# rapidsai/cudf

Measured on AMD Instinct MI355X. Metric: rows/sec + achieved HBM GB/s: 1e9-row int64 sort & hash-join, 1/2/4/8 GPU, higher is better.
Workload: dtype int64; 1 GPU; 1e+09-row int64 radix sort (cudf::sort, keys only); rows_per_gpu=1000000000, algo=0, parallelism=1 GPU

## Files before the change

### cudf_amd/csrc/gx_sort.hip

```cpp
#include "gx_common.hpp"
#include <cstdlib>
#include <type_traits>
#include <vector>
#include "gx_scan.hpp"

namespace gx {
namespace sort {

constexpr int BINS       = 256;
constexpr int MAX_PASSES = 8;
constexpr int BT         = 512;
constexpr int NW         = BT / GX_WAVE;
constexpr int NRANGE     = 8;

constexpr int CS_MAXBITS = 15;
constexpr int NB2MAX     = 1024;
constexpr int NB9        = 512;

struct HybridPlan {
  int32_t attempt;
  int32_t ok;
  int32_t shift0;
  int32_t shift2, bits2;
  int32_t nlocal;
  int32_t lshift[MAX_PASSES], lbits[MAX_PASSES];
  int32_t need_hist;
  int32_t cell_max;
  int32_t overflow;
  int32_t bad;
  uint32_t plan2_done;
  unsigned long long or_mask, nor_mask;
  uint32_t list_tile0[2][NRANGE + 1];
  uint32_t seg_tile0[2][BINS + 1];
  uint32_t seg_start[2][BINS], seg_count[2][BINS];
  uint32_t max_cell;
  uint32_t hist0[BINS], gbin0[BINS];
  uint32_t rh0[NRANGE][BINS];
  uint32_t rhist[NRANGE][MAX_PASSES][BINS];
  unsigned long long fold_or;
  int32_t fold;
  unsigned long long fold_x;
  alignas(128) uint32_t todo_count;
  uint32_t todo_pad[31];
  int32_t big;
  int32_t lsd_mode;
  uint32_t nbig;
  uint32_t big_pad;
  unsigned long long lsd_n;
  uint32_t bigbucket[BINS];
  uint32_t bigcnt[BINS], bigkeys[BINS];
  uint32_t biglist0[BINS], bigx0[BINS];
  uint32_t cbase[BINS], ccap[BINS];
};
__device__ __forceinline__ uint32_t cell_cap(const HybridPlan& hy, uint32_t b) { return hy.ccap[b] ? hy.ccap[b] : (uint32_t)hy.cell_max; }
__device__ __forceinline__ uint32_t cell_slot(const HybridPlan& hy, uint32_t b, uint32_t d2)
{
  return hy.ccap[b] ? hy.cbase[b] + d2 * hy.ccap[b] : ((b << hy.bits2) + d2) * (uint32_t)hy.cell_max;
}
static inline size_t cell_slack(int cell_max) { return (size_t)(6.0 * __builtin_sqrt((double)cell_max)) + 64 + 16 + 2; }

struct FastPlan {
  int32_t state;
  int32_t cs_bits;
  uint32_t cs_fail;
  uint32_t cs_groups;
  unsigned long long cs_base;
  int32_t fail;
  int32_t stride;
  int32_t hist_ready;
  int32_t slots_ready;
  uint32_t samp[NRANGE][BINS];
  uint32_t slot0[NRANGE][BINS];
  uint32_t cap0[NRANGE][BINS];
  uint32_t reg_tile0[BINS * NRANGE + 1];
  uint32_t reg_start[BINS * NRANGE], reg_count[BINS * NRANGE];
  alignas(128) uint32_t cur0[NRANGE][BINS];
  uint32_t forced_masks;
  unsigned long long forced_or, forced_nor;
  uint32_t ext, nreg;
  uint32_t slot_total;
  uint32_t* x_tile0;
  const uint32_t* x_start;
  const uint32_t* x_count;
  const uint32_t* x_bucket;
};

struct alignas(128) Counter {
  uint32_t v;
  uint32_t pad[31];
};
struct SortCounters {
  Counter tickets[MAX_PASSES];
  Counter ctr[2][NRANGE];
};

constexpr int SP_NSAMP = 16384;
// ... 25 lines not shown
};
struct SpCell {
  unsigned long long lo, w;
  uint32_t mlow;
  int nsh;
};
__device__ __forceinline__ SpCell sp_cell_of(const SplitPlan& sp, uint32_t b) { return SpCell{sp.lo[b], sp.w[b], sp.mlow[b], sp.nsh[b]}; }
__device__ __forceinline__ bool sp_narrow(const SplitPlan& sp, uint32_t b, int bits2) { return sp.nw[b] != 0u && sp.nw[b] <= (1u << bits2) && !sp.eq[b]; }
__device__ __forceinline__ uint32_t sp_cell(uint32_t frac, uint32_t nc) { return __umulhi(frac, nc); }
template <int CL2>
__device__ __forceinline__ uint32_t sp_fine(uint32_t frac, uint32_t nc) { return __umulhi(frac, nc << CL2) & ((1u << CL2) - 1u); }
__device__ __forceinline__ uint32_t sp_warp(uint32_t frac, const uint2* wt)
{
  const uint2 e = wt[frac >> SP_PSH];
  return e.x + __umulhi(frac << (32 - SP_PSH), e.y);
}
__device__ __forceinline__ uint32_t sp_frac(const SpCell& c, unsigned long long key)
{
  const unsigned long long rel = key > c.lo ? key - c.lo : 0ull;
  if (rel >= c.w) return 0xFFFFFFFFu;
  const uint32_t x2 = c.nsh == 63 ? 0u : ((uint32_t)((rel << (33 - c.nsh)) >> 32) & ~1u);
  return x2 + __umulhi(x2, c.mlow);
}
__device__ __forceinline__ uint32_t sp_lut_cell(unsigned long long rel, uint32_t lut_log, uint32_t lshift)
{
  if (lut_log) {
    if (rel == 0) return 0;
    const int e      = 63 - __builtin_clzll(rel);
    const uint32_t m = e >= 6 ? (uint32_t)(rel >> (e - 6)) & 63u : (uint32_t)(rel << (6 - e)) & 63u;
    return (uint32_t)e * 64u + m;
  }
  const unsigned long long c = rel >> lshift;
  return c < (unsigned long long)(SP_NLUT - 1) ? (uint32_t)c : (uint32_t)(SP_NLUT - 1);
}
struct SpLutF {
  unsigned long long nmin, pmin;
  uint32_t nsh, psh;
};
__device__ __forceinline__ SpLutF sp_lutf_of(const SplitPlan& sp) { return SpLutF{sp.f_nmin, sp.f_pmin, sp.f_nsh, sp.f_psh}; }
template <int KIND, int F2 = -1>
__device__ __forceinline__ uint32_t sp_lut_cell_k(unsigned long long key, unsigned long long kmin, uint32_t form, uint32_t lshift, const SpLutF& f)
{
  if (F2 == 1 || (F2 < 0 && form == 2u)) {
    const bool pos             = key >= f.pmin;
    const unsigned long long o = pos ? f.pmin : f.nmin;
    const unsigned long long c = (key > o ? key - o : 0ull) >> (pos ? f.psh : f.nsh);
    return (pos ? (uint32_t)(SP_NLUT / 2) : 0u) + (c < (unsigned long long)(SP_NLUT / 2 - 1) ? (uint32_t)c : (uint32_t)(SP_NLUT / 2 - 1));
  }
  return sp_lut_cell(key >= kmin ? key - kmin : 0ull, form, lshift);
}
template <int KIND, int F2 = -1>
__device__ __forceinline__ uint32_t sp_bucket(const unsigned long long* __restrict__ tab, const uint16_t* __restrict__ lut, unsigned long long key,
                                              uint32_t nsp, unsigned long long kmin, uint32_t lut_log, uint32_t lshift, const SpLutF& lf)
{
  const uint32_t wd            = lut[sp_lut_cell_k<KIND, F2>(key, kmin, lut_log, lshift, lf)];
  uint32_t b                   = wd & 0x1FFu;
  if (wd & 0x8000u) return b;
  const uint32_t inside = (wd >> 9) & 63u;
  if (inside <= 4u) {
    while (b < nsp && tab[b] <= key) ++b;
    return b;
  }
  uint32_t lo = b, hi = inside == 63u ? nsp : b + inside;
  while (lo < hi) {
    const uint32_t mid = (lo + hi) >> 1;
    if (tab[mid] <= key) lo = mid + 1; else hi = mid;
  }
  return lo;
}

struct SortPlan {
  uint32_t hist[MAX_PASSES][BINS];
  uint32_t gbin[MAX_PASSES][BINS];
  int32_t pass_skip[MAX_PASSES];
  int32_t pass_src[MAX_PASSES];
  int32_t pass_dst[MAX_PASSES];
  int32_t num_active;
  int32_t status;
  HybridPlan hy;
  SortCounters cnt;
  FastPlan hf;
  SplitPlan sp;
};

struct Digit0 {
  int shift, fsh;
  uint32_t dm, fhi;
  template <typename KeyT>
  __device__ __forceinline__ uint32_t operator()(KeyT k) const { return ((uint32_t)(k >> shift) & dm) | ((uint32_t)(k >> fsh) & fhi); }
};
__device__ __forceinline__ Digit0 digit0_of(const HybridPlan& hy, int key_bits)
{
  return hy.fold ? Digit0{hy.shift0, key_bits - 8, 0x7Fu, 0x80u} : Digit0{hy.shift0, 0, 0xFFu, 0u};
}
__device__ __forceinline__ int fold_height(unsigned long long fold_or, unsigned long long V, int key_bits)
{
  if (!((V >> (key_bits - 1)) & 1ull)) return 0;
  const int h = fold_or ? 64 - __builtin_clzll(fold_or) : 0;
  return (h >= 7 && h <= key_bits - 10) ? h : 0;
}

template <typename KeyT, int KIND>
__global__ void __launch_bounds__(BT) k_hist_all(const KeyT* __restrict__ in, int64_t n, KeyT desc_mask,
                                                 SortPlan* plan, int64_t range_rows, const KeyT* __restrict__ inB = nullptr)
{
  if (plan->hy.ok && !plan->hy.lsd_mode) return;
  if (plan->hy.lsd_mode) {
    in         = inB;
    n          = (int64_t)plan->hy.lsd_n;
    range_rows = div_up(div_up(n, (int64_t)NRANGE), (int64_t)GX_WAVE) * GX_WAVE;
  }
  const int range      = blockIdx.x % NRANGE;
  const int64_t rbegin = (int64_t)range * range_rows < n ? (int64_t)range * range_rows : n;
  const int64_t rend   = (range == NRANGE - 1) ? n : (rbegin + range_rows < n ? rbegin + range_rows : n);
  constexpr int NPASS = sizeof(KeyT);
  __shared__ uint32_t s_hist[NPASS * BINS];
  __shared__ unsigned long long s_fold[NW];
  for (int i = threadIdx.x; i < NPASS * BINS; i += BT) s_hist[i] = 0;
  __syncthreads();
  const unsigned lane  = lane_id();
  KeyT fold            = 0;
  constexpr int UNROLL = 4;
  const int64_t stride = (int64_t)(gridDim.x / NRANGE) * BT * UNROLL;
  for (int64_t i0 = rbegin + (int64_t)(blockIdx.x / NRANGE) * BT * UNROLL + threadIdx.x; i0 < rend; i0 += stride) {
    KeyT raw[UNROLL];
#pragma unroll
    for (int u = 0; u < UNROLL; ++u) {
      const int64_t i = i0 + (int64_t)u * BT;
      raw[u]          = (i < rend) ? in[i] : KeyT(0);
    }
#pragma unroll
    for (int u = 0; u < UNROLL; ++u) {
      const int64_t i = i0 + (int64_t)u * BT;
      if (i < rend) {
        const KeyT k          = to_sortable<KeyT, KIND>(raw[u], desc_mask);
        if (KIND == K_SIGNED) fold |= (KeyT)(raw[u] ^ (KeyT)(KeyT(0) - (KeyT)(raw[u] >> (8 * sizeof(KeyT) - 1))));
        const uint64_t active = ballot(true);
        const int leader      = __builtin_ctzll(active);
#pragma unroll
        for (int p = 0; p < NPASS; ++p) {
          const uint32_t d  = (uint32_t)(k >> (8 * p)) & 0xFFu;
          const uint32_t d0 = __builtin_amdgcn_readfirstlane(d);
          const uint64_t same = ballot(d == d0);
          if (same == active) {
            if ((int)lane == leader) atomicAdd(&s_hist[p * BINS + d0], (uint32_t)__builtin_popcountll(active));
          } else if (__builtin_popcountll(same) >= 8) {
            if ((int)lane == leader) atomicAdd(&s_hist[p * BINS + d0], (uint32_t)__builtin_popcountll(same));
            else if (d != d0) atomicAdd(&s_hist[p * BINS + d], 1u);
          } else {
            atomicAdd(&s_hist[p * BINS + d], 1u);
          }
        }
      }
    }
  }
  if (KIND == K_SIGNED) {
    const unsigned long long wf = wave_reduce((unsigned long long)fold, [](unsigned long long x, unsigned long long y) { return x | y; });
    if (lane == 0) s_fold[threadIdx.x / GX_WAVE] = wf;
  }
  __syncthreads();
  if (KIND == K_SIGNED && threadIdx.x == 0) {
    unsigned long long f = 0;
    for (int k = 0; k < NW; ++k) f |= s_fold[k];
    if (f & ~__hip_atomic_load(&plan->hy.fold_or, __ATOMIC_RELAXED, __HIP_MEMORY_SCOPE_AGENT)) atomicOr(&plan->hy.fold_or, f);
  }
  for (int i = threadIdx.x; i < NPASS * BINS; i += BT) {
// ... 2435 lines not shown
      }
    }
    __syncthreads();
    uint32_t q  = s_misc[0];
    uint32_t jt = s_misc[1];
    if constexpr (LVL == 2) {
      q  = (uint32_t)__builtin_amdgcn_readfirstlane((int)q);
      jt = (uint32_t)__builtin_amdgcn_readfirstlane((int)jt);
    }
    seg               = q / NRANGE;
    if (LVL == 2 && !hy.bigbucket[seg]) return;
    base              = (int64_t)hf.reg_start[q] + (int64_t)jt * TILE;
    const int64_t rem = (int64_t)hf.reg_count[q] - (int64_t)jt * TILE;
    nvalid            = (int)(rem < (int64_t)TILE ? rem : (int64_t)TILE);
  } else {
    const uint32_t nreg    = hf.nreg;
    const uint32_t* rtile0 = hf.x_tile0;
    if (v >= (int64_t)rtile0[nreg]) return;
    for (uint32_t q = tid; q < nreg; q += BT) {
      const uint32_t lo = rtile0[q], hi = rtile0[q + 1];
      if ((int64_t)lo <= v && v < (int64_t)hi) {
        s_misc[0] = q;
        s_misc[1] = (uint32_t)(v - lo);
      }
    }
    __syncthreads();
    uint32_t q  = s_misc[0];
    uint32_t jt = s_misc[1];
    if constexpr (LVL == 2) {
      q  = (uint32_t)__builtin_amdgcn_readfirstlane((int)q);
      jt = (uint32_t)__builtin_amdgcn_readfirstlane((int)jt);
    }
    seg               = hf.x_bucket[q];
    if (LVL == 2 && !hy.bigbucket[seg]) return;
    base              = (int64_t)hf.x_start[q] + (int64_t)jt * TILE;
    const int64_t rem = (int64_t)hf.x_count[q] - (int64_t)jt * TILE;
    nvalid            = (int)(rem < (int64_t)TILE ? rem : (int64_t)TILE);
  }
  const uint32_t dmask = LVL == 0 ? 0xFFu : ((1u << hy.bits2) - 1u);
  const Digit0 dig     = LVL == 0 ? digit0_of(hy, (int)(8 * sizeof(KeyT))) : Digit0{hy.shift2, 0, dmask, 0u};
  const uint32_t cap_s  = LVL >= 1 ? cell_cap(hy, seg) : 0u;
  const uint32_t base_s = LVL >= 1 ? cell_slot(hy, seg, 0u) : 0u;
  SpCell spc{0ull, 1ull, 0u, 63};
  if (split) {
    if (plan->sp.eq[seg]) {
      if (LVL == 2) return;
      if (tid == 0) s_misc[2] = atomicAdd(&cellcur[seg * NB2MAX], (uint32_t)nvalid);
      __syncthreads();
      const int64_t dst0 = (int64_t)hy.gbin0[seg] + (int64_t)s_misc[2];
#pragma unroll
      for (int j = 0; j < KPT; ++j) {
        const int idx = j * BT + (int)tid;
        if (idx < nvalid) fin[dst0 + idx] = in[base + idx];
      }
      return;
    }
    spc = sp_cell_of(plan->sp, seg);
    if (tid < (unsigned)SP_NPIECE) s_wt[tid] = plan->sp.wt[seg][tid];
  }
  const uint32_t spnc = split ? plan->sp.nc[seg] : 1u;
  auto spdig          = [&](KeyT k) -> uint32_t {
    if constexpr (sizeof(KeyT) == 8) return sp_cell(sp_warp(sp_frac(spc, (unsigned long long)k), s_wt), spnc);
    else return dig(k);
  };
  if (split && sp_narrow(plan->sp, seg, hy.bits2)) {
    if (LVL == 2) return;
    for (int b = tid; b < NB; b += BT) s_cnt[b] = 0;
    __syncthreads();
#pragma unroll
    for (int j = 0; j < KPT; ++j) {
      const int idx   = j * BT + (int)tid;
      const bool live = idx < nvalid;
      const KeyT k    = to_sortable<KeyT, KIND>(in[base + (live ? idx : 0)], desc_mask);
      (void)lds_rank(s_cnt, spdig(k), live);
    }
    __syncthreads();
    for (int b = tid; b < NB; b += BT) {
      const uint32_t c = s_cnt[b];
      if (c) atomicAdd(&cellcur[seg * NB2MAX + b], c);
    }
    return;
  }

  KeyT key[KPT];
  if (nvalid == TILE) {
#pragma unroll
    for (int j = 0; j < KPT; ++j) key[j] = in[base + j * BT + (int)tid];
  } else {
#pragma unroll
    for (int j = 0; j < KPT; ++j) {
      const int idx = j * BT + (int)tid;
      key[j]        = in[base + (idx < nvalid ? idx : 0)];
    }
  }
  for (int b = tid; b < NB; b += BT) s_cnt[b] = 0;
  if constexpr (LVL == 0 && KIND == K_FTOTAL) {
    bool unclean = false;
#pragma unroll
    for (int j = 0; j < KPT; ++j) unclean |= float_unclean<KeyT>(key[j]);
    if (unclean) hf.fail = 1;
  }
  if (LVL == 0) {
    auto mform = [&](KeyT k) -> KeyT {
      if constexpr (KIND == K_FTOTAL) return to_sortable<KeyT, KIND>(k, KeyT(0));
      else return k;
    };
    KeyT vor = mform(key[0]), vnor = (KeyT)~mform(key[0]);
#pragma unroll
    for (int j = 1; j < KPT; ++j) {
      vor |= mform(key[j]);
      vnor |= (KeyT)~mform(key[j]);
    }
    const unsigned long long wo = wave_reduce((unsigned long long)vor, [](unsigned long long x, unsigned long long y) { return x | y; });
    const unsigned long long wn = wave_reduce((unsigned long long)vnor, [](unsigned long long x, unsigned long long y) { return x | y; });
    if (lane_id() == 0) {
      s_red[tid / GX_WAVE]      = wo;
      s_red[NW + tid / GX_WAVE] = wn;
    }
    if (KIND == K_SIGNED && hy.fold) {
      KeyT vf = 0;
#pragma unroll
      for (int j = 0; j < KPT; ++j) vf |= (KeyT)(key[j] ^ (KeyT)(KeyT(0) - (KeyT)(key[j] >> (8 * sizeof(KeyT) - 1))));
      const unsigned long long wf = wave_reduce((unsigned long long)vf, [](unsigned long long x, unsigned long long y) { return x | y; });
      if (lane_id() == 0 && (wf & ~__hip_atomic_load(&hy.fold_x, __ATOMIC_RELAXED, __HIP_MEMORY_SCOPE_AGENT))) atomicOr(&hy.fold_x, wf);
    }
  }
  __syncthreads();
  if (LVL == 0 && tid == 0) {
    unsigned long long o = 0, no = 0;
    for (int k = 0; k < NW; ++k) {
      o |= s_red[k];
      no |= s_red[NW + k];
    }
    if (o & ~__hip_atomic_load(&hy.or_mask, __ATOMIC_RELAXED, __HIP_MEMORY_SCOPE_AGENT)) atomicOr(&hy.or_mask, o);
    if (no & ~__hip_atomic_load(&hy.nor_mask, __ATOMIC_RELAXED, __HIP_MEMORY_SCOPE_AGENT)) atomicOr(&hy.nor_mask, no);
  }
  constexpr bool RANK16 = sizeof(KeyT) == 4;
  uint32_t packed[RANK16 ? KPT / 2 : KPT];
  if constexpr (RANK16) {
#pragma unroll
    for (int j = 0; j < KPT / 2; ++j) packed[j] = 0;
  }
  auto rank_all = [&](auto&& digf) {
#pragma unroll
    for (int j = 0; j < KPT; ++j) {
      const bool live  = j * BT + (int)tid < nvalid;
      const KeyT k     = to_sortable<KeyT, KIND>(key[j], desc_mask);
      const uint32_t d = digf(k);
      const uint32_t r = lds_rank(s_cnt, d, live);
      if constexpr (RANK16) packed[j >> 1] |= r << (16 * (j & 1));
      else packed[j] = (d << 16) | r;
    }
  };
  if (split) rank_all(spdig); else rank_all(dig);
  __syncthreads();
  uint32_t c[BPT], g[BPT], sbase[BPT], scap[BPT];
  bool skip[BPT];
  uint32_t csum = 0;
#pragma unroll
  for (int k = 0; k < BPT; ++k) {
    const uint32_t bin = tid * BPT + k;
    c[k] = g[k] = sbase[k] = scap[k] = 0;
    skip[k] = false;
    if (bin < (uint32_t)NB) {
      c[k] = s_cnt[bin];
      if (LVL == 0) {
        sbase[k] = hf.slot0[seg][bin];
        scap[k]  = hf.cap0[seg][bin];
        if (c[k]) g[k] = atomicAdd(&hf.cur0[seg][bin], c[k]);
      } else if (LVL == 1 && bin <= dmask) {
        sbase[k] = base_s + bin * cap_s;
        scap[k]  = cap_s;
        if (c[k]) g[k] = atomicAdd(&cellcur[seg * NB2MAX + bin], c[k]);
      } else if (LVL == 2 && bin <= dmask) {
        const uint32_t total = cellcur[seg * NB2MAX + bin];
        if (total > cap_s) {
          sbase[k] = xoff[seg * NB2MAX + bin];
          scap[k]  = total;
          if (c[k]) g[k] = atomicAdd(&rescur[seg * NB2MAX + bin], c[k]);
        } else {
          skip[k] = true;
        }
      }
      csum += c[k];
    }
  }
  uint32_t st = block_exclusive_scan<BT>(csum, 0u, SumOp(), s_scan, (uint32_t*)nullptr);
  bool spilled = false;
#pragma unroll
  for (int k = 0; k < BPT; ++k) {
    const uint32_t bin = tid * BPT + k;
    if (bin < (uint32_t)NB) {
      if (c[k] && !skip[k] && g[k] + c[k] > scap[k]) spilled = true;
      s_cnt[bin]   = st;
      s_delta[bin] = sbase[k] + g[k] - st;
      s_limit[bin] = sbase[k] + scap[k];
      st += c[k];
    }
  }
  if (spilled) {
    if (LVL == 0) hf.fail = 1;
    else if (LVL == 1) {
      if (!__hip_atomic_load(&hy.overflow, __ATOMIC_RELAXED, __HIP_MEMORY_SCOPE_AGENT)) atomicExch(&hy.overflow, 1);
    } else atomicExch(&hy.bad, 2);
  }
  __syncthreads();
#pragma unroll
  for (int j = 0; j < KPT; ++j) {
    if (j * BT + (int)tid < nvalid) {
      if constexpr (RANK16) {
        const uint32_t d = dig(to_sortable<KeyT, KIND>(key[j], desc_mask));
        s_keys[s_cnt[d] + ((packed[j >> 1] >> (16 * (j & 1))) & 0xFFFFu)] = key[j];
      } else {
        s_keys[s_cnt[packed[j] >> 16] + (packed[j] & 0xFFFFu)] = key[j];
      }
    }
  }
  __syncthreads();
  auto write_all = [&](auto&& digf) {
#pragma unroll
    for (int j = 0; j < KPT; ++j) {
      const int i = j * BT + (int)tid;
      if (i < nvalid) {
        const KeyT k       = s_keys[i];
        const uint32_t d   = digf(to_sortable<KeyT, KIND>(k, desc_mask));
        const uint32_t dst = s_delta[d] + (uint32_t)i;
        if (dst < s_limit[d]) out[dst] = k;
      }
    }
  };
  if (split) write_all(spdig); else write_all(dig);
}

template <typename KeyT, int KIND, int LVL, int NBL>
__global__ void __launch_bounds__(BT, 4) k_hf_scatter(const KeyT* __restrict__ in, KeyT* __restrict__ out, KeyT desc_mask, SortPlan* plan,
                                                     uint32_t* __restrict__ cellcur, uint32_t cellcap, int64_t n, KeyT* __restrict__ fin = nullptr,
                                                     uint32_t ntiles = 0)
{
  if constexpr (LVL == 2) {
    if (plan->hf.state != 3 || !(plan->hy.ok && plan->hy.lsd_mode)) return;
    for (uint32_t t = blockIdx.x; t < ntiles; t += gridDim.x) {
      hf_scatter_tile<KeyT, KIND, LVL, NBL>(in, out, desc_mask, plan, cellcur, n, fin, (int64_t)t, (int64_t)ntiles);
      __syncthreads();
    }
  } else {
    hf_scatter_tile<KeyT, KIND, LVL, NBL>(in, out, desc_mask, plan, cellcur, n, fin, (int64_t)blockIdx.x, (int64_t)gridDim.x);
  }
}

constexpr int SP_KPT  = 14;
constexpr int SP_TILE = BT * SP_KPT;
constexpr size_t sp_level0_lds() { return (size_t)SP_TILE * 8 + (size_t)(3 * BINS + 16 + 4) * 4 + (size_t)2 * NW * 8 + (size_t)BINS * 8 + (size_t)SP_NLUT * 2 + (size_t)SP_TILE; }
template <int KIND, int F2>
__global__ void __launch_bounds__(BT, 4) k_sp_level0(const uint64_t* __restrict__ in, uint64_t* __restrict__ out, uint64_t desc_mask, SortPlan* plan, int64_t n)
{
  constexpr int KPT = SP_KPT, TILE = SP_TILE;
  extern __shared__ __attribute__((aligned(16))) char smem[];
  uint64_t* s_keys  = reinterpret_cast<uint64_t*>(smem);
  uint32_t* s_cnt   = reinterpret_cast<uint32_t*>(smem + (size_t)TILE * 8);
  uint32_t* s_delta = s_cnt + BINS;
  uint32_t* s_limit = s_delta + BINS;
  uint32_t* s_scan  = s_limit + BINS;
  uint32_t* s_misc  = s_scan + 16;
  unsigned long long* s_red = reinterpret_cast<unsigned long long*>(s_misc + 4);
  unsigned long long* s_tab = s_red + 2 * NW;
  uint16_t* s_lut   = reinterpret_cast<uint16_t*>(s_tab + BINS);
  uint8_t* s_bid    = reinterpret_cast<uint8_t*>(s_lut + SP_NLUT);
  HybridPlan& hy      = plan->hy;
  FastPlan& hf        = plan->hf;
  const SplitPlan& sp = plan->sp;
  if (hf.state != 1 || !sp.on || !hf.slots_ready) return;
  if ((sp.lut_log == 2u) != (F2 == 1)) return;
  const unsigned tid = threadIdx.x;
  const int64_t v    = xcd_swizzle((int64_t)blockIdx.x, (int64_t)gridDim.x);
  const int64_t per  = (int64_t)gridDim.x / NRANGE;
  const uint32_t seg = (per > 0 && v / per < NRANGE - 1) ? (uint32_t)(v / per) : (uint32_t)(NRANGE - 1);
  const int64_t base = v * TILE;
  const int nvalid   = (int)(n - base < (int64_t)TILE ? n - base : (int64_t)TILE);
  uint64_t key[KPT];
  if (nvalid == TILE) {
#pragma unroll
    for (int j = 0; j < KPT; ++j) key[j] = in[base + j * BT + (int)tid];
  } else {
#pragma unroll
    for (int j = 0; j < KPT; ++j) {
      const int idx = j * BT + (int)tid;
      key[j]        = in[base + (idx < nvalid ? idx : 0)];
    }
  }
  for (int b = tid; b < BINS; b += BT) {
    s_cnt[b] = 0;
    s_tab[b] = sp.tab[b];
  }
  for (int i = tid; i < SP_NLUT; i += BT) s_lut[i] = sp.lut[i];
  if constexpr (KIND == K_FTOTAL) {
    bool unclean = false;
#pragma unroll
    for (int j = 0; j < KPT; ++j) unclean |= float_unclean<uint64_t>(key[j]);
    if (unclean) hf.fail = 1;
  }
  {
    auto mform = [&](uint64_t k) -> uint64_t {
      if constexpr (KIND == K_FTOTAL) return to_sortable<uint64_t, KIND>(k, 0ull);
      else return k;
    };
    uint64_t vor = mform(key[0]), vnor = ~mform(key[0]);
#pragma unroll
    for (int j = 1; j < KPT; ++j) {
      vor |= mform(key[j]);
      vnor |= ~mform(key[j]);
    }
    const unsigned long long wo = wave_reduce((unsigned long long)vor, [](unsigned long long x, unsigned long long y) { return x | y; });
    const unsigned long long wn = wave_reduce((unsigned long long)vnor, [](unsigned long long x, unsigned long long y) { return x | y; });
    if (lane_id() == 0) {
      s_red[tid / GX_WAVE]      = wo;
      s_red[NW + tid / GX_WAVE] = wn;
    }
  }
  __syncthreads();
  if (tid == 0) {
    unsigned long long o = 0, no = 0;
    for (int k = 0; k < NW; ++k) {
      o |= s_red[k];
      no |= s_red[NW + k];
    }
    if (o & ~__hip_atomic_load(&hy.or_mask, __ATOMIC_RELAXED, __HIP_MEMORY_SCOPE_AGENT)) atomicOr(&hy.or_mask, o);
    if (no & ~__hip_atomic_load(&hy.nor_mask, __ATOMIC_RELAXED, __HIP_MEMORY_SCOPE_AGENT)) atomicOr(&hy.nor_mask, no);
  }
  const uint32_t nsp = sp.nsp, lut_log = sp.lut_log, lshift = sp.lshift;
  const unsigned long long kmin = sp.kmin;
  const SpLutF lf               = sp_lutf_of(sp);
  uint32_t packed[KPT];
#pragma unroll
  for (int j = 0; j < KPT; ++j) packed[j] = 0;
  const uint32_t steps = sp.lut_steps;
  if (steps <= 4u) {
#pragma unroll
    for (int j = 0; j < KPT; ++j) {
      const uint64_t k = to_sortable<uint64_t, KIND>(key[j], desc_mask);
      packed[j]        = (uint32_t)s_lut[sp_lut_cell_k<KIND, F2>(k, kmin, lut_log, lshift, lf)] & 0x1FFu;
    }
    for (uint32_t st = 0; st < steps; ++st) {
#pragma unroll
      for (int j = 0; j < KPT; ++j) {
        const uint64_t k  = to_sortable<uint64_t, KIND>(key[j], desc_mask);
        const uint32_t bb = packed[j];
        packed[j]         = bb + ((bb < nsp && s_tab[bb] <= k) ? 1u : 0u);
      }
    }
#pragma unroll
    for (int j = 0; j < KPT; ++j) {
      const bool live  = j * BT + (int)tid < nvalid;
      const uint32_t d = packed[j];
      const uint32_t r = lds_rank(s_cnt, d, live);
      packed[j]        = (d << 16) | r;
    }
  } else {
#pragma unroll
    for (int j = 0; j < KPT; ++j) {
      const bool live  = j * BT + (int)tid < nvalid;
      const uint64_t k = to_sortable<uint64_t, KIND>(key[j], desc_mask);
      const uint32_t d = sp_bucket<KIND, F2>(s_tab, s_lut, k, nsp, kmin, lut_log, lshift, lf);
      const uint32_t r = lds_rank(s_cnt, d, live);
      packed[j]        = (d << 16) | r;
    }
  }
  __syncthreads();
  uint32_t c = 0, g = 0, sbase = 0, scap = 0;
  if (tid < (unsigned)BINS) {
    c     = s_cnt[tid];
    sbase = hf.slot0[seg][tid];
    scap  = hf.cap0[seg][tid];
    if (c) g = atomicAdd(&hf.cur0[seg][tid], c);
  }
  uint32_t st = block_exclusive_scan<BT>(c, 0u, SumOp(), s_scan, (uint32_t*)nullptr);
  if (tid < (unsigned)BINS) {
    if (c && g + c > scap) hf.fail = 1;
    s_cnt[tid]   = st;
    s_delta[tid] = sbase + g - st;
    s_limit[tid] = sbase + scap;
  }
  __syncthreads();
#pragma unroll
  for (int j = 0; j < KPT; ++j) {
    if (j * BT + (int)tid < nvalid) {
      const uint32_t d   = packed[j] >> 16;
      const uint32_t pos = s_cnt[d] + (packed[j] & 0xFFFFu);
      s_keys[pos]        = key[j];
      s_bid[pos]         = (uint8_t)d;
    }
  }
  __syncthreads();
#pragma unroll
  for (int j = 0; j < KPT; ++j) {
    const int i = j * BT + (int)tid;
    if (i < nvalid) {
      const uint32_t d   = s_bid[i];
      const uint32_t dst = s_delta[d] + (uint32_t)i;
      if (dst < s_limit[d]) out[dst] = s_keys[i];
    }
  }
}

static thread_local int g_algorithm = 0;
static thread_local int g_order_mode = 0;

struct Profile {
  bool enabled = false;
  bool created = false;
  int level    = 1;
  int npass    = 0;
  hipEvent_t ev[2 * MAX_PASSES + 2];
  hipEvent_t hev[5];
  bool hybrid_marked = false;
};
constexpr int PROF_SLOTS = 64;
static thread_local Profile g_profs[PROF_SLOTS];
static thread_local int g_prof_slot = 0;
#define g_prof g_profs[g_prof_slot]
static inline void prof_mark(int idx, hipStream_t s)
{
  if (g_prof.enabled && g_prof.level == 1) (void)hipEventRecord(g_prof.ev[idx], s);
}
static inline void prof_mark_h(int idx, hipStream_t s)
{
  if (g_prof.enabled && (g_prof.level == 1 || idx <= 1)) (void)hipEventRecord(g_prof.hev[idx], s);
}
static thread_local int g_hybrid = 1;
static thread_local int g_lbw    = 16;
static thread_local int g_msd_kpt = 16;

template <typename KeyT>
constexpr int kpt_for(bool has_val)
{
  return (sizeof(KeyT) == 8 && has_val) ? 10 : 16;
}

template <typename KeyT, bool HAS_VAL, int KPT>
constexpr size_t pass_lds_bytes()
{
  return (size_t)BT * KPT * sizeof(KeyT) + (HAS_VAL ? (size_t)BT * KPT * 4 : 0) +
         (size_t)(NW * BINS + BINS + 16 + 4) * 4;
}

struct HybridCfg {
  bool on;
  int cl2;
  int bits2;
  int kpt;
  int cl2_alt;
};
static thread_local int g_cell = 0;
static inline unsigned local_sort_grid(int cells) { return (unsigned)(cells < 4096 ? cells : 4096); }
static thread_local int g_place_grid = 0;
static inline unsigned local_place_grid(int cells) { return (unsigned)((g_place_grid > 0 && g_place_grid < cells) ? g_place_grid : cells); }
enum class Role { primary, fallback };
constexpr int FALLBACK_WGS_PER_CU = 16;
static inline unsigned role_grid(const Device& dev, Role role, int64_t want)
{
  const int64_t cap = (int64_t)FALLBACK_WGS_PER_CU * dev.cus;
  return (unsigned)((role == Role::fallback && want > cap) ? cap : want);
}
template <typename KeyT, int KIND, bool HAS_VAL>
static HybridCfg hybrid_cfg(int64_t n, bool iota_payload, int algo)
{
  HybridCfg c{false, 14, 8, HAS_VAL ? 10 : g_msd_kpt, 0};
  if (sizeof(KeyT) != 8 || (HAS_VAL && !iota_payload) || algo != 0 || !g_hybrid || n < (1ll << 22)) return c;
  const bool small_ok = KIND != K_FLOAT;
  c.cl2 = (small_ok && g_cell != 16384 && (double)n / (double)(1 << 17) <= 0.955 * 8192.0) ? 13 : 14;
  if (g_cell == 8192 && small_ok) c.cl2 = 13;
  const double cell = (double)(1 << c.cl2);
  const int maxb2   = small_ok ? 9 : 8;
  int B = 9;
  while (B < 8 + maxb2 && (double)n / (double)(1ull << B) > 0.955 * cell) ++B;
  if ((double)n / (double)(1ull << B) > 0.97 * cell) return c;
  c.bits2 = B - 8;
  c.on    = true;
  if (HAS_VAL && c.cl2 == 13 && g_cell == 0) c.cl2_alt = 14;
  return c;
}

struct FastCfg {
  bool on;
// ... 33 lines not shown
template <typename KeyT, int KIND, bool HAS_VAL>
int sort_impl(const void* keys_in, void* keys_out, const int32_t* vals_in, int32_t* vals_out, int64_t n,
              int descending, bool radix_nan_rule, void* tmp, size_t* tmp_bytes, hipStream_t stream)
{
  constexpr int KPT   = kpt_for<KeyT>(HAS_VAL);
  constexpr int TILE  = BT * KPT;
  constexpr int NPASS = sizeof(KeyT);
  if (n < 0 || tmp_bytes == nullptr) return GX_EINVAL;
  if (n > 0x7FFFFFFFll) return GX_EINVAL;
  const int64_t ntiles = n > 0 ? div_up(n, TILE) : 0;
  const int algo       = g_algorithm;

  Carver c(tmp);
  SortPlan* plan             = c.take<SortPlan>(1);
  unsigned long long* status = nullptr;
  uint32_t* tile_hist        = nullptr;
  uint32_t* partials         = nullptr;
  HybridCfg hc     = hybrid_cfg<KeyT, KIND, HAS_VAL>(n, vals_in == nullptr, algo);
  const FastCfg fc = fast_cfg<KeyT, KIND, HAS_VAL>(n, algo, hc.on);
  const size_t fc_cells = fc.on ? (size_t)n + (size_t)n / 16 + ((size_t)BINS << fc.bits2_max) * cell_slack(1 << 13) + 65536 : 0;
  if (fc.on && hc.on && hc.cl2 == 14 && (((size_t)BINS << hc.bits2) << 14) > fc_cells + (size_t)n / 4) hc.on = false;
  const bool try_hybrid = hc.on;
  const int hyb_kpt     = hc.kpt;
  const int nb1         = hc.bits2 > 8 ? NB9 : BINS;
  uint32_t* base1 = c.take<uint32_t>((size_t)NRANGE * NB2MAX);
  const bool cells = try_hybrid || fc.on;
  uint32_t* hist2 = cells ? c.take<uint32_t>((size_t)4 * BINS * NB2MAX) : nullptr;
  uint32_t* base2 = cells ? hist2 + BINS * NB2MAX : nullptr;
  uint32_t* xoff  = cells ? hist2 + 2 * BINS * NB2MAX : nullptr;
  uint32_t* todo  = cells ? c.take<uint32_t>((size_t)BINS * NB2MAX) : nullptr;
  uint32_t* biglist = fc.on ? c.take<uint32_t>((size_t)2 * BIG_LIST) : nullptr;
  const int64_t msd_tile     = (int64_t)BT * hyb_kpt;
  const int64_t msd_ntiles   = n > 0 ? div_up(n, msd_tile) : 0;
  const int64_t status_tiles = (msd_ntiles > ntiles ? msd_ntiles : ntiles) + BINS + 2 * NRANGE;
  const size_t status_words  = (size_t)status_tiles * (try_hybrid ? nb1 : BINS);
  if (algo != 1) {
    status = c.take<unsigned long long>(status_words);
  } else {
    tile_hist = c.take<uint32_t>((size_t)ntiles * BINS);
    partials  = c.take<uint32_t>(scan::partials_count(ntiles * BINS));
  }
  size_t padded = try_hybrid ? ((size_t)BINS << hc.bits2) << (hc.cl2_alt ? hc.cl2_alt : hc.cl2) : 0;
  if (fc_cells > padded) padded = fc_cells;
  const size_t nb_buf = padded > (size_t)n ? padded : (size_t)n;
  KeyT* kb_scratch = c.take<KeyT>(nb_buf);
  KeyT* slot0_buf  = fc.on ? c.take<KeyT>(fc.slot_rows) : nullptr;
  KeyT* ka_scratch = keys_out ? nullptr : c.take<KeyT>((size_t)n);
  uint32_t* vb     = HAS_VAL ? c.take<uint32_t>(nb_buf) : nullptr;
  if (tmp == nullptr) {
    *tmp_bytes = c.total();
    return 0;
  }
  if (*tmp_bytes < c.total()) return GX_ETMP;
  if (n > 0 && (keys_in == nullptr || (HAS_VAL && vals_out == nullptr))) return GX_EINVAL;
  if (n > 0 && keys_in == keys_out) return GX_EINVAL;

  GX_HIP_TRY(hipMemsetAsync(plan, 0, sizeof(SortPlan), stream));
  if (n == 0) return 0;
  Device dev;
  GX_HIP_TRY(device(&dev));
  if (algo != 1 && !fc.on) GX_HIP_TRY(hipMemsetAsync(status, 0, status_words * sizeof(unsigned long long), stream));
  const size_t hist2_bytes = (size_t)4 * BINS * NB2MAX * sizeof(uint32_t);
  if (cells && !fc.on) GX_HIP_TRY(hipMemsetAsync(hist2, 0, hist2_bytes, stream));
  const int64_t range_rows = try_hybrid ? div_up(msd_ntiles, NRANGE) * msd_tile : div_up(ntiles, NRANGE) * TILE;

  const KeyT desc_mask = descending ? KeyT(~KeyT(0)) : KeyT(0);
  g_prof.npass = NPASS;
  int64_t hblocks = div_up(n, (int64_t)BT * 8);
  if (hblocks > 2048) hblocks = 2048;
  hblocks = div_up(hblocks, NRANGE) * NRANGE;
  prof_mark(0, stream);
  g_prof.hybrid_marked = false;
  bool cursor_marked = false;
  constexpr int CK = (KIND == K_FLOAT) ? (int)K_FTOTAL : KIND;
  if constexpr ((sizeof(KeyT) == 8 || sizeof(KeyT) == 4) && !HAS_VAL && (KIND != K_FLOAT || sizeof(KeyT) == 8)) {
    if (fc.on) {
      constexpr int FT = BT * hf_kpt<KeyT>();
      constexpr int MIN_SHIFT2 = 8;
      constexpr int WORD_BYTES = (int)sizeof(typename PlaceWord<KeyT, CK, HAS_VAL>::type);
      const int64_t ftiles  = div_up(n, (int64_t)FT);
      const int64_t frange  = (ftiles / NRANGE) * FT;
      auto lds_hf = [&](int nb) { return (size_t)FT * sizeof(KeyT) + (size_t)(3 * nb + 16 + 4) * 4 + (size_t)2 * NW * 8; };
      typedef void (*HfK)(const KeyT*, KeyT*, KeyT, SortPlan*, uint32_t*, uint32_t, int64_t, KeyT*, uint32_t);
      HfK kf0 = k_hf_scatter<KeyT, CK, 0, 8>;
      HfK kf1 = fc.bits2_max <= 8 ? (HfK)k_hf_scatter<KeyT, CK, 1, 8> : (fc.bits2_max == 9 ? (HfK)k_hf_scatter<KeyT, CK, 1, 9> : (HfK)k_hf_scatter<KeyT, CK, 1, 10>);
      HfK kf2 = fc.bits2_max <= 8 ? (HfK)k_hf_scatter<KeyT, CK, 2, 8> : (fc.bits2_max == 9 ? (HfK)k_hf_scatter<KeyT, CK, 2, 9> : (HfK)k_hf_scatter<KeyT, CK, 2, 10>);
      const int nbf = fc.bits2_max <= 8 ? 256 : (1 << fc.bits2_max);
      const int64_t step = (int64_t)fc.stride * HF_CHUNK;
      int64_t sblocks    = div_up(div_up(n, step), (int64_t)4 * 4);
      if (sblocks > 2048) sblocks = 2048;
      const KeyT* kin = static_cast<const KeyT*>(keys_in);
      KeyT* bufA      = keys_out ? static_cast<KeyT*>(keys_out) : ka_scratch;
      hipLaunchKernelGGL((k_hf_sample<KeyT, CK, false>), dim3((unsigned)sblocks), dim3(256), 0, stream, kin, n, desc_mask, plan, fc.stride, frange,
                         reinterpret_cast<uint4*>(hist2), hist2_bytes / sizeof(uint4));
      hipLaunchKernelGGL(k_hf_plan, dim3(1), dim3(BINS), 0, stream, plan, 0, (int)(8 * sizeof(KeyT)), n, fc.bits2, 1 << 13, fc.stride, frange, FT,
                         (unsigned long long)fc.slot_rows, g_cursor_margin, MIN_SHIFT2, fc.bits2_max, 0ull, CK == K_SIGNED ? 1 : 0, (KIND == K_FLOAT) ? 0 : g_counting);
      {
        GX_HIP_TRY(launch_lds(dev, (k_cs_count<KeyT, CK>), dim3(256), dim3(CS_BT), (size_t)4 << CS_MAXBITS, stream, kin, n, desc_mask, plan, hist2));
        hipLaunchKernelGGL(k_cs_scan, dim3(1), dim3(CS_BT), 0, stream, plan, (const uint32_t*)hist2, base2, xoff, n, NPASS);
        hipLaunchKernelGGL((k_cs_fill<KeyT, CK>), dim3(4096), dim3(256), 0, stream, bufA, n, desc_mask, (const SortPlan*)plan, (const uint32_t*)base2,
                           (const uint32_t*)xoff);
      }
      hipLaunchKernelGGL((k_hf_sample<KeyT, CK, true>), dim3((unsigned)sblocks), dim3(256), 0, stream, kin, n, desc_mask, plan, fc.stride, frange);
      const int allow_split = (sizeof(KeyT) == 8 && g_split) ? 1 : 0;
      hipLaunchKernelGGL(k_hf_plan, dim3(1), dim3(BINS), 0, stream, plan, 1, (int)(8 * sizeof(KeyT)), n, fc.bits2, 1 << 13, fc.stride, frange, FT,
                         (unsigned long long)fc.slot_rows, g_cursor_margin, MIN_SHIFT2, fc.bits2_max, 0ull, 0, 0, allow_split);
      int64_t ftiles_s = 0;
      if constexpr (sizeof(KeyT) == 8) {
        if (allow_split) {
          ftiles_s               = div_up(n, (int64_t)SP_TILE);
          const int64_t frange_s = (ftiles_s / NRANGE) * SP_TILE;
          GX_HIP_TRY(launch_lds(dev, (k_sp_plan<CK>), dim3(1), dim3(1024), (size_t)SP_NSAMP * 8, stream, kin, n, (uint64_t)desc_mask, plan, fc.bits2_max));
          hipLaunchKernelGGL((k_sp_sample<CK>), dim3((unsigned)(sblocks > 1024 ? 1024 : sblocks)), dim3(256), 0, stream, kin, n, (uint64_t)desc_mask, plan, fc.stride, frange_s);
          hipLaunchKernelGGL(k_hf_plan, dim3(1), dim3(BINS), 0, stream, plan, 1, (int)(8 * sizeof(KeyT)), n, fc.bits2, 1 << 13, fc.stride, frange_s, FT,
                             (unsigned long long)fc.slot_rows, g_cursor_margin, MIN_SHIFT2, fc.bits2_max, 0ull, 0, 0, allow_split);
        }
      }
      prof_mark(1, stream);
      prof_mark_h(0, stream);
      GX_HIP_TRY(launch_lds(dev, kf0, dim3((unsigned)ftiles), dim3(BT), lds_hf(256), stream, kin, slot0_buf, desc_mask, plan, hist2, 1u << 13, n, (KeyT*)nullptr, 0u));
      if constexpr (sizeof(KeyT) == 8) {
        if (allow_split)
        {
          GX_HIP_TRY(launch_lds(dev, (k_sp_level0<CK, 0>), dim3((unsigned)ftiles_s), dim3(BT), sp_level0_lds(), stream, kin, slot0_buf, (uint64_t)desc_mask, plan, n));
          GX_HIP_TRY(launch_lds(dev, (k_sp_level0<CK, 1>), dim3((unsigned)ftiles_s), dim3(BT), sp_level0_lds(), stream, kin, slot0_buf, (uint64_t)desc_mask, plan, n));
        }
      }
      hipLaunchKernelGGL(k_hf_plan, dim3(1), dim3(BINS), 0, stream, plan, 2, (int)(8 * sizeof(KeyT)), n, fc.bits2, 1 << 13, fc.stride, frange, FT,
                         (unsigned long long)fc.slot_rows, g_cursor_margin, MIN_SHIFT2, fc.bits2_max, (unsigned long long)nb_buf);
      prof_mark_h(1, stream);
      GX_HIP_TRY(launch_lds(dev, kf1, dim3((unsigned)(ftiles + NRANGE * BINS)), dim3(BT), lds_hf(nbf), stream, slot0_buf, kb_scratch, desc_mask, plan, hist2, 1u << 13, n, bufA, 0u));
      prof_mark_h(2, stream);
      hipLaunchKernelGGL(k_plan2, dim3(BINS), dim3(GX_WAVE), 0, stream, plan, hist2, base2, NPASS, 1);
      prof_mark_h(3, stream);
      if constexpr (sizeof(KeyT) == 8) {
        if (allow_split)
          hipLaunchKernelGGL((k_sp_fill<CK>), dim3(BINS, SP_FILL_Y), dim3(256), 0, stream, bufA, (uint64_t)desc_mask, (const SortPlan*)plan, (const uint32_t*)base2);
      }
      GX_HIP_TRY(launch_lds(dev, (k_local_place<KeyT, CK, HAS_VAL, 13>), dim3(local_place_grid(BINS << fc.bits2)), dim3((1 << 13) / 16),
                                 place_lds_bytes(13, WORD_BYTES), stream, kb_scratch, bufA, (const uint32_t*)nullptr, (uint32_t*)nullptr, desc_mask, plan, hist2,
                                 base2, todo, g_exp, 1));
      GX_HIP_TRY(launch_lds(dev, (k_local_sort<uint64_t, CK, HAS_VAL, 13, KeyT>), dim3(local_sort_grid(BINS << fc.bits2_max)), dim3((1 << 13) / 16),
                                 ((size_t)8 << 13) + (size_t)(((1 << 13) / 16 / GX_WAVE) * BINS + 32 + 2 * BINS) * 4, stream, (const KeyT*)kb_scratch, bufA,
                                 (const uint32_t*)nullptr, (uint32_t*)nullptr, (uint64_t)desc_mask, plan, hist2, base2, g_exp, 1, (const uint32_t*)todo));
      prof_mark_h(4, stream);
      g_prof.hybrid_marked = g_prof.enabled;
      cursor_marked        = true;
      hipLaunchKernelGGL(k_big_plan, dim3(1), dim3(BINS), 0, stream, plan, (unsigned long long)(fc.slot_rows / 2));
      hipLaunchKernelGGL(k_big_cells, dim3(BINS), dim3(GX_WAVE), 0, stream, (const SortPlan*)plan, (const uint32_t*)hist2, xoff, biglist);
      GX_HIP_TRY(launch_lds(dev, kf2, dim3(role_grid(dev, Role::fallback, ftiles + NRANGE * BINS)), dim3(BT), lds_hf(nbf), stream, slot0_buf, kb_scratch, desc_mask, plan,
                            hist2, 1u << 13, n, bufA, (uint32_t)(ftiles + NRANGE * BINS)));
      hipLaunchKernelGGL(k_hf_clear_status, dim3(2048), dim3(256), 0, stream, plan, reinterpret_cast<uint4*>(status), status_words / 2);
    }
  }
  if constexpr (sizeof(KeyT) == 8) {
    if (try_hybrid) {
      constexpr size_t pay   = HAS_VAL ? 4 : 0;
      constexpr bool STABLE  = KIND == K_FLOAT || HAS_VAL;
      constexpr bool SMALLOK = KIND != K_FLOAT;
      constexpr int SKPT     = HAS_VAL ? 10 : 16;
      auto lds_msd = [&](int kpt, int nb) {
        const int wrows = STABLE ? ((HAS_VAL && nb == NB9) ? NW / 2 : NW) : 2;
        return (size_t)BT * kpt * (sizeof(KeyT) + pay) + (size_t)(wrows * nb + 2 * nb + 16 + 4) * 4;
      };
      auto lds_loc = [&](int cl2) { return ((size_t)sizeof(KeyT) << cl2) + (size_t)(((1 << cl2) / 16 / GX_WAVE) * BINS + 32 + 2 * BINS) * 4; };
      typedef void (*MsdK)(MsdArgs);
      MsdK kmsd0 = HAS_VAL ? (MsdK)k_msd_pass<KeyT, KIND, HAS_VAL, 10, 4, 8>
                           : (hyb_kpt == 8 ? (MsdK)k_msd_pass<KeyT, KIND, HAS_VAL, 8, 4, 8>
                                           : (hyb_kpt == 12 ? (MsdK)k_msd_pass<KeyT, KIND, HAS_VAL, 12, 4, 8> : (MsdK)k_msd_pass<KeyT, KIND, HAS_VAL, 16, 4, 8>));
      MsdK kmsd1 = kmsd0;
      auto kloc  = k_local_sort<KeyT, KIND, HAS_VAL, 14>;
      int ls_bt  = (1 << 14) / 16;
      int kpt1 = hyb_kpt;
      if constexpr (SMALLOK) {
        if (hc.bits2 > 8) {
          kmsd1 = (MsdK)k_msd_pass<KeyT, KIND, HAS_VAL, SKPT, 4, 9>;
          kpt1  = SKPT;
        }
        if constexpr (!HAS_VAL) if (g_lbw != 4 && hyb_kpt == 16) {
          kmsd0 = g_lbw == 8 ? (MsdK)k_msd_pass<KeyT, KIND, HAS_VAL, 16, 8, 8> : (MsdK)k_msd_pass<KeyT, KIND, HAS_VAL, 16, 16, 8>;
          if (hc.bits2 > 8) kmsd1 = g_lbw == 8 ? (MsdK)k_msd_pass<KeyT, KIND, HAS_VAL, 16, 8, 9> : (MsdK)k_msd_pass<KeyT, KIND, HAS_VAL, 16, 16, 9>;
          else kmsd1 = kmsd0;
        }
        if (hc.cl2 == 13) {
          kloc  = k_local_sort<KeyT, KIND, HAS_VAL, 13>;
          ls_bt = (1 << 13) / 16;
        }
      }
      if (kpt1 != hyb_kpt) return GX_EINTERNAL;
      const Role lb_role = (fc.on && SMALLOK) ? Role::fallback : Role::primary;
      bool msd_multi     = false;
      if constexpr (!HAS_VAL && SMALLOK) {
        if (lb_role == Role::fallback && hyb_kpt == 16 && g_lbw == 16) {
          kmsd0 = (MsdK)k_msd_pass<KeyT, KIND, HAS_VAL, 16, 16, 8, true>;
          kmsd1 = hc.bits2 > 8 ? (MsdK)k_msd_pass<KeyT, KIND, HAS_VAL, 16, 16, 9, true> : kmsd0;
          msd_multi = true;
        }
      }
      const Role msd_role = msd_multi ? Role::fallback : Role::primary;
      hipLaunchKernelGGL((k_hy_hist<KeyT, KIND, true>), dim3((unsigned)hblocks), dim3(BT), 0, stream,
                         static_cast<const KeyT*>(keys_in), n, desc_mask, plan, range_rows);
      hipLaunchKernelGGL(k_hy_plan, dim3(1), dim3(BINS), 0, stream, plan, 0, (int)(8 * sizeof(KeyT)), n, hc.bits2, 1 << hc.cl2,
                         HAS_VAL ? hc.cl2 : 0, range_rows, (int)msd_tile, base1, 0, KIND == K_SIGNED ? 1 : 0);
      hipLaunchKernelGGL((k_hy_hist<KeyT, KIND, false>), dim3((unsigned)hblocks), dim3(BT), 0, stream,
                         static_cast<const KeyT*>(keys_in), n, desc_mask, plan, range_rows);
      hipLaunchKernelGGL(k_hy_plan, dim3(1), dim3(BINS), 0, stream, plan, 1, (int)(8 * sizeof(KeyT)), n, hc.bits2, 1 << hc.cl2,
                         HAS_VAL ? hc.cl2 : 0, range_rows, (int)msd_tile, base1, hc.cl2_alt ? (1 << hc.cl2_alt) : 0);
      if (!cursor_marked) prof_mark(1, stream);
      KeyT* bufA = keys_out ? static_cast<KeyT*>(keys_out) : ka_scratch;
// ... 797 lines not shown
```

Baseline: 91.65 billion rows/s.

## Merge level-0 scatter launches and use wide nontemporal loads in upper levels

The three level-0 kernel launches (the bit-scatter and two split-LUT variants, two of which early-exited) become one k_level0 kernel that picks the path per block from plan state. This removes empty launches and their gaps. In hf_scatter_tile for levels 1 and up, 64-bit keys are now loaded as 16-byte vectors with nontemporal hints when the tile is full and aligned, to cut load instruction count and cache pollution on streaming reads. The merged kernel always reserves the larger LDS footprint, which may lower occupancy for the bit-scatter path.

```diff
diff --git a/cudf_amd/csrc/gx_sort.hip b/cudf_amd/csrc/gx_sort.hip
--- a/cudf_amd/csrc/gx_sort.hip
+++ b/cudf_amd/csrc/gx_sort.hip
@@ -1,4 +1,5 @@
 #include "gx_common.hpp"
+#include <cstddef>
 #include <cstdlib>
 #include <type_traits>
 #include <vector>
@@ -12,6 +13,14 @@
 constexpr int BT         = 512;
 constexpr int NW         = BT / GX_WAVE;
 constexpr int NRANGE     = 8;
+
+typedef unsigned long long u64x2 __attribute__((ext_vector_type(2)));
+template <bool NT, typename T>
+__device__ __forceinline__ T stream_load(const T* p)
+{
+  if constexpr (NT) return __builtin_nontemporal_load(p);
+  else return *p;
+}
 
 constexpr int CS_MAXBITS = 15;
 constexpr int NB2MAX     = 1024;
@@ -203,6 +212,7 @@
   FastPlan hf;
   SplitPlan sp;
 };
+static_assert(offsetof(SortPlan, sp) + offsetof(SplitPlan, lut_log) == 166812, "SplitPlan::lut_log moved: update SP_LUT_FORM_BYTE in the test");
 
 struct Digit0 {
   int shift, fsh;
@@ -2804,15 +2814,27 @@
     return;
   }
 
+  constexpr bool NTB = LVL >= 1;
+  constexpr bool W16 = LVL >= 1 && sizeof(KeyT) == 8;
   KeyT key[KPT];
-  if (nvalid == TILE) {
-#pragma unroll
-    for (int j = 0; j < KPT; ++j) key[j] = in[base + j * BT + (int)tid];
+  if (W16 && nvalid == TILE && (reinterpret_cast<uintptr_t>(in + base) & 15u) == 0u) {
+    if constexpr (W16) {
+      const u64x2* in2 = reinterpret_cast<const u64x2*>(in + base);
+#pragma unroll
+      for (int j = 0; j < KPT / 2; ++j) {
+        const u64x2 q  = stream_load<NTB>(&in2[j * BT + (int)tid]);
+        key[2 * j]     = (KeyT)q.x;
+        key[2 * j + 1] = (KeyT)q.y;
+      }
+    }
+  } else if (nvalid == TILE) {
+#pragma unroll
+    for (int j = 0; j < KPT; ++j) key[j] = stream_load<NTB>(&in[base + j * BT + (int)tid]);
   } else {
 #pragma unroll
     for (int j = 0; j < KPT; ++j) {
       const int idx = j * BT + (int)tid;
-      key[j]        = in[base + (idx < nvalid ? idx : 0)];
+      key[j]        = stream_load<NTB>(&in[base + (idx < nvalid ? idx : 0)]);
     }
   }
   for (int b = tid; b < NB; b += BT) s_cnt[b] = 0;
@@ -2974,7 +2996,8 @@
 constexpr int SP_TILE = BT * SP_KPT;
 constexpr size_t sp_level0_lds() { return (size_t)SP_TILE * 8 + (size_t)(3 * BINS + 16 + 4) * 4 + (size_t)2 * NW * 8 + (size_t)BINS * 8 + (size_t)SP_NLUT * 2 + (size_t)SP_TILE; }
 template <int KIND, int F2>
-__global__ void __launch_bounds__(BT, 4) k_sp_level0(const uint64_t* __restrict__ in, uint64_t* __restrict__ out, uint64_t desc_mask, SortPlan* plan, int64_t n)
+__device__ __forceinline__ void sp_level0_tile(const uint64_t* __restrict__ in, uint64_t* __restrict__ out, uint64_t desc_mask, SortPlan* plan, int64_t n,
+                                               int64_t vblock, int64_t ntiles)
 {
   constexpr int KPT = SP_KPT, TILE = SP_TILE;
   extern __shared__ __attribute__((aligned(16))) char smem[];
@@ -2991,11 +3014,9 @@
   HybridPlan& hy      = plan->hy;
   FastPlan& hf        = plan->hf;
   const SplitPlan& sp = plan->sp;
-  if (hf.state != 1 || !sp.on || !hf.slots_ready) return;
-  if ((sp.lut_log == 2u) != (F2 == 1)) return;
   const unsigned tid = threadIdx.x;
-  const int64_t v    = xcd_swizzle((int64_t)blockIdx.x, (int64_t)gridDim.x);
-  const int64_t per  = (int64_t)gridDim.x / NRANGE;
+  const int64_t v    = xcd_swizzle(vblock, ntiles);
+  const int64_t per  = ntiles / NRANGE;
   const uint32_t seg = (per > 0 && v / per < NRANGE - 1) ? (uint32_t)(v / per) : (uint32_t)(NRANGE - 1);
   const int64_t base = v * TILE;
   const int nvalid   = (int)(n - base < (int64_t)TILE ? n - base : (int64_t)TILE);
@@ -3121,6 +3142,24 @@
       const uint32_t dst = s_delta[d] + (uint32_t)i;
       if (dst < s_limit[d]) out[dst] = s_keys[i];
     }
+  }
+}
+
+template <typename KeyT, int KIND>
+__global__ void __launch_bounds__(BT, 4)
+k_level0(const KeyT* __restrict__ in, KeyT* __restrict__ out, KeyT desc_mask, SortPlan* plan, uint32_t* __restrict__ cellcur, int64_t n, int64_t nt_bit, int64_t nt_sp)
+{
+  const FastPlan& hf = plan->hf;
+  if (hf.state != 1) return;
+  const int64_t b = (int64_t)blockIdx.x;
+  if (!plan->sp.on) {
+    if (b < nt_bit) hf_scatter_tile<KeyT, KIND, 0, 8>(in, out, desc_mask, plan, cellcur, n, (KeyT*)nullptr, b, nt_bit);
+    return;
+  }
+  if constexpr (sizeof(KeyT) == 8) {
+    if (!hf.slots_ready || b >= nt_sp) return;
+    if (plan->sp.lut_log == 2u) sp_level0_tile<KIND, 1>(in, out, desc_mask, plan, n, b, nt_sp);
+    else sp_level0_tile<KIND, 0>(in, out, desc_mask, plan, n, b, nt_sp);
   }
 }
 
@@ -3320,7 +3359,6 @@
       const int64_t frange  = (ftiles / NRANGE) * FT;
       auto lds_hf = [&](int nb) { return (size_t)FT * sizeof(KeyT) + (size_t)(3 * nb + 16 + 4) * 4 + (size_t)2 * NW * 8; };
       typedef void (*HfK)(const KeyT*, KeyT*, KeyT, SortPlan*, uint32_t*, uint32_t, int64_t, KeyT*, uint32_t);
-      HfK kf0 = k_hf_scatter<KeyT, CK, 0, 8>;
       HfK kf1 = fc.bits2_max <= 8 ? (HfK)k_hf_scatter<KeyT, CK, 1, 8> : (fc.bits2_max == 9 ? (HfK)k_hf_scatter<KeyT, CK, 1, 9> : (HfK)k_hf_scatter<KeyT, CK, 1, 10>);
       HfK kf2 = fc.bits2_max <= 8 ? (HfK)k_hf_scatter<KeyT, CK, 2, 8> : (fc.bits2_max == 9 ? (HfK)k_hf_scatter<KeyT, CK, 2, 9> : (HfK)k_hf_scatter<KeyT, CK, 2, 10>);
       const int nbf = fc.bits2_max <= 8 ? 256 : (1 << fc.bits2_max);
@@ -3356,13 +3394,10 @@
       }
       prof_mark(1, stream);
       prof_mark_h(0, stream);
-      GX_HIP_TRY(launch_lds(dev, kf0, dim3((unsigned)ftiles), dim3(BT), lds_hf(256), stream, kin, slot0_buf, desc_mask, plan, hist2, 1u << 13, n, (KeyT*)nullptr, 0u));
-      if constexpr (sizeof(KeyT) == 8) {
-        if (allow_split)
-        {
-          GX_HIP_TRY(launch_lds(dev, (k_sp_level0<CK, 0>), dim3((unsigned)ftiles_s), dim3(BT), sp_level0_lds(), stream, kin, slot0_buf, (uint64_t)desc_mask, plan, n));
-          GX_HIP_TRY(launch_lds(dev, (k_sp_level0<CK, 1>), dim3((unsigned)ftiles_s), dim3(BT), sp_level0_lds(), stream, kin, slot0_buf, (uint64_t)desc_mask, plan, n));
-        }
+      {
+        const int64_t tiles0 = ftiles_s > ftiles ? ftiles_s : ftiles;
+        const size_t lds0    = ftiles_s > 0 && sp_level0_lds() > lds_hf(256) ? sp_level0_lds() : lds_hf(256);
+        GX_HIP_TRY(launch_lds(dev, (k_level0<KeyT, CK>), dim3((unsigned)tiles0), dim3(BT), lds0, stream, kin, slot0_buf, desc_mask, plan, hist2, n, ftiles, ftiles_s));
       }
       hipLaunchKernelGGL(k_hf_plan, dim3(1), dim3(BINS), 0, stream, plan, 2, (int)(8 * sizeof(KeyT)), n, fc.bits2, 1 << 13, fc.stride, frange, FT,
                          (unsigned long long)fc.slot_rows, g_cursor_margin, MIN_SHIFT2, fc.bits2_max, (unsigned long long)nb_buf);
```

Result: faster. 94.32 billion rows/s (median of 6 runs) (+2.9%).
